# noiseinspacechannel/NIS-SAR-AMTIGMTI-Video

Hardware: AMD Instinct MI355X
Metric: focused SAR frames/sec (CSA focus, complex64) (higher is better)
Workload: dtype c64 (phase arguments f64)

## Files before the change

nis-sar-amtigmti-video_amd/csrc/api_csa.hip:

```cpp
#include "api_ctx.h"
#include "csa_kernels.h"
#include "general.h"

#include <cmath>
#include <cstdlib>
#include <string>
#include <vector>

using namespace sarx;

struct sarx_plan {
    sarx_ctx* ctx = nullptr;
    int n_az = 0, n_rg = 0;
    unsigned flags = 0;
    sarx_radar_params p{};
    int az_s = 0;
    int az_w = 32;
    int az_w_alone = 0;
    int az_impl = 1;
    int az_wpb = 4;
    int look = 0;
    float* look_slot = nullptr;
    float* look_part = nullptr;
    const float2* ati_s1 = nullptr; const float* ati_thr = nullptr; float ati_frac = 0.f; double ati_cal = 0.0;
    float *ati_phase = nullptr, *ati_m1 = nullptr, *ati_dm = nullptr; int ati_keep_image = 0;
    double2* ati_part = nullptr; int ati_nparts = 0;
    int ati_w = 32;
    float* max_slot = nullptr;
    bool az_nt = false;
    int slab_tiles = 0;
    double2 *c1 = nullptr, *c2 = nullptr, *c3 = nullptr;
    float2* buf_b = nullptr;
    float2* buf_a = nullptr;
    float2 *h_in = nullptr, *h_out = nullptr;
    static constexpr int PIPE = 2;
    float2 *pipe_in[PIPE] = {}, *pipe_out[PIPE] = {};
    int pipe_dl[PIPE] = {-1, -1};
    void* pipe_host[PIPE] = {};
    int pipe_next = 0;
    uint64_t bytes = 0;
    int mark_start = -1, mark_stop = -1;
    unsigned long long* stamp = nullptr;
    GeneralCsa* gen = nullptr;
};

static bool is_pow2(int n) { return n > 0 && (n & (n - 1)) == 0; }
static int ilog2(int n) { int l = 0; while ((1 << l) < n) ++l; return l; }

extern "C" {

static int sarx_csa_plan_create_impl(sarx_ctx* c, int n_az, int n_rg, const sarx_radar_params* prm, unsigned flags, sarx_plan** out) {
    NEED_CTX(c);
    if (!out || !prm) return fail(c, SARX_ERR_INVALID, "NULL argument");
    *out = nullptr;
    if (n_az < 2 || n_rg < 2 || n_az > 2 * TW_MAX || n_rg > 2 * TW_MAX)
        return fail(c, SARX_ERR_UNSUPPORTED, "n_az=%d n_rg=%d: sizes must be in [2, %d]", n_az, n_rg, 2 * TW_MAX);
    if (flags & ~(SARX_OUT_RG_MAJOR | SARX_FUSE_RANGE)) return fail(c, SARX_ERR_INVALID, "unknown plan flags 0x%x", flags);
    const bool general = !is_pow2(n_az) || !is_pow2(n_rg) || n_az < 16 || n_rg < 16 || n_az > TW_MAX || n_rg > TW_MAX;
    if (!(prm->sample_rate_hz > 0) || !(prm->prf_hz > 0) || !(prm->platform_speed_mps > 0) ||
        !(prm->wavelength_m > 0) || prm->chirp_rate_hz_s == 0.0)
        return fail(c, SARX_ERR_INVALID, "radar parameters must be positive (chirp rate non-zero)");
    sarx_plan* p = new sarx_plan();
    p->ctx = c; p->n_az = n_az; p->n_rg = n_rg; p->flags = flags; p->p = *prm;
    if (general) {
        std::string err;
        p->gen = general_csa_create(n_az, n_rg, prm, c->tw_all, err, true, c->cus);
        if (!p->gen) { delete p; return fail(c, SARX_ERR_UNSUPPORTED, "n_az=%d n_rg=%d: %s", n_az, n_rg, err.c_str()); }
        p->bytes = general_csa_bytes(p->gen);
        if (flags & SARX_OUT_RG_MAJOR) {
            hipError_t e2 = hipMalloc(&p->buf_a, (size_t)n_az * n_rg * sizeof(float2));
            if (e2 != hipSuccess) { int rc = fail(c, SARX_ERR_NOMEM, "hipMalloc: %s", hipGetErrorString(e2)); sarx_csa_plan_destroy(p); return rc; }
            p->bytes += (size_t)n_az * n_rg * sizeof(float2);
        }
        *out = p;
        return SARX_OK;
    }
    p->az_s = (n_az <= 128) ? n_az : (1 << (ilog2(n_az) / 2));
    p->az_w = (n_rg % 32 == 0) ? 32 : 16;
    p->az_nt = (size_t)n_az * n_rg * sizeof(float2) >= ((size_t)1 << 29);
    if (const char* e = getenv("SARX_AZ_NT")) p->az_nt = atoi(e) != 0;
    if (const char* e = getenv("SARX_SLAB_MIB")) {
        const double mib = atof(e);
        const double tile_mib = (double)p->az_s * n_rg * sizeof(float2) / (1024.0 * 1024.0);
        if (mib > 0 && p->az_s != n_az) {
            int q = (int)(mib / tile_mib);
            if (q < 1) q = 1;
            if (q > n_az / p->az_s) q = n_az / p->az_s;
            p->slab_tiles = q;
        }
    }
    if (const char* e = getenv("SARX_AZ_W")) { const int w = atoi(e); if ((w == 16 || w == 32 || w == 64) && n_rg % w == 0) p->az_w = w; }
    else if (n_rg % 64 == 0 && (size_t)n_az * n_rg * sizeof(float2) >= ((size_t)1 << 31)) p->az_w_alone = 64;
    if (const char* e = getenv("SARX_AZ_IMPL")) p->az_impl = atoi(e) != 0;
    if (const char* e = getenv("SARX_AZ_WAVES")) { const int w = atoi(e); if (w == 1 || w == 4) p->az_wpb = w; }

    const double lam = prm->wavelength_m, Kr = prm->chirp_rate_hz_s, Vr = prm->platform_speed_mps, Rref = prm->range_ref_m;
    const double fa_step = 1.0 / ((double)n_az * (1.0 / prm->prf_hz));
    std::vector<double2> c1(n_az), c2(n_az), c3(n_az);
    for (int i = 0; i < n_az; ++i) {
        const int ks = (i < n_az / 2) ? i : i - n_az;
        const double fa = (double)ks * fa_step;
        const double u = lam * fa / (2.0 * Vr);
        double arg = 1.0 - u * u;
        if (arg < 0) arg = 1e-9;
        const double D = sqrt(arg);
        const double Cs = 1.0 / D - 1.0;
        const double tau_ref = 2.0 * Rref / (C_LIGHT * D);
        c1[i] = make_double2(-0.5 * Kr * Cs, tau_ref);
        c2[i] = make_double2(0.5 / (Kr * (1.0 + Cs)), 2.0 * Rref * Cs / C_LIGHT);
        c3[i] = make_double2(C_LIGHT * D / lam, -0.5 * Kr * Cs * (1.0 + Cs));
    }
    const size_t tb = (size_t)n_az * sizeof(double2), img = (size_t)n_az * n_rg * sizeof(float2);
    auto bail = [&](hipError_t e, const char* what) {
        int rc = fail(c, e == hipErrorOutOfMemory ? SARX_ERR_NOMEM : SARX_ERR_DEVICE, "%s: %s", what, hipGetErrorString(e));
        sarx_csa_plan_destroy(p);
        return rc;
    };
    hipError_t e;
    if ((e = hipMalloc(&p->c1, tb)) != hipSuccess) return bail(e, "hipMalloc c1");
    if ((e = hipMalloc(&p->c2, tb)) != hipSuccess) return bail(e, "hipMalloc c2");
    if ((e = hipMalloc(&p->c3, tb)) != hipSuccess) return bail(e, "hipMalloc c3");
    if ((e = hipMemcpy(p->c1, c1.data(), tb, hipMemcpyHostToDevice)) != hipSuccess) return bail(e, "upload c1");
    if ((e = hipMemcpy(p->c2, c2.data(), tb, hipMemcpyHostToDevice)) != hipSuccess) return bail(e, "upload c2");
    if ((e = hipMemcpy(p->c3, c3.data(), tb, hipMemcpyHostToDevice)) != hipSuccess) return bail(e, "upload c3");
    if ((e = hipMalloc(&p->buf_b, img)) != hipSuccess) return bail(e, "hipMalloc scratch image");
    p->bytes = 3 * tb + img;
    if (flags & SARX_OUT_RG_MAJOR) {
        if ((e = hipMalloc(&p->buf_a, img)) != hipSuccess) return bail(e, "hipMalloc second scratch image");
        p->bytes += img;
    }
    *out = p;
    return SARX_OK;
}
int sarx_csa_plan_create(sarx_ctx* c, int n_az, int n_rg, const sarx_radar_params* prm, unsigned flags, sarx_plan** out) {
    return guarded(c, [&] { return sarx_csa_plan_create_impl(c, n_az, n_rg, prm, flags, out); });
}

int sarx_csa_plan_destroy(sarx_plan* p) {
    if (!p) return SARX_OK;
    hipSetDevice(p->ctx->device);
    sync_all_lanes(p->ctx);
    general_csa_destroy(p->gen);
    hipFree(p->c1); hipFree(p->c2); hipFree(p->c3);
    hipFree(p->ati_part);
    hipFree(p->buf_a); hipFree(p->buf_b); hipFree(p->h_in); hipFree(p->h_out); hipFree(p->look_part);
    for (int i = 0; i < sarx_plan::PIPE; ++i)
        if (p->pipe_dl[i] >= 0 && p->pipe_dl[i] < sarx_ctx::DL_SLOTS) { sarx_memcpy_d2h_end(p->ctx, p->pipe_dl[i]); p->pipe_dl[i] = -1; }
    if (p->ctx->dl_stream) hipStreamSynchronize(p->ctx->dl_stream);
    for (int i = 0; i < sarx_plan::PIPE; ++i) { hipFree(p->pipe_in[i]); hipFree(p->pipe_out[i]); }
    delete p;
    return SARX_OK;
}

int sarx_csa_plan_mark_range(sarx_plan* p, int slot_start, int slot_stop) {
    if (!p) return fail(nullptr, SARX_ERR_INVALID, "plan is NULL");
    if (slot_start >= N_EVENTS || slot_stop >= N_EVENTS) return fail(p->ctx, SARX_ERR_INVALID, "event slot out of range");
    p->mark_start = slot_start; p->mark_stop = slot_stop;
    return SARX_OK;
}

int sarx_csa_plan_stamp_range(sarx_plan* p, uint64_t* d_pair) {
    if (!p) return fail(nullptr, SARX_ERR_INVALID, "plan is NULL");
    if (((uintptr_t)d_pair) & 7) return fail(p->ctx, SARX_ERR_INVALID, "the stamp pair must be 8-byte aligned");
    p->stamp = reinterpret_cast<unsigned long long*>(d_pair);
    return SARX_OK;
}

int sarx_csa_plan_set_look_slot(sarx_plan* p, int looks, float* d_slot) {
    if (!p) return fail(nullptr, SARX_ERR_INVALID, "plan is NULL");
    sarx_ctx* c = p->ctx;
    hipSetDevice(c->device);
    if (!d_slot) { p->look_slot = nullptr; return SARX_OK; }
    if (p->gen) return fail(c, SARX_ERR_UNSUPPORTED, "the fused stack slot exists for power-of-two plans only (use sarx_multilook_dev)");
    if (looks < 1 || (looks & (looks - 1)) || looks > p->az_w || p->n_az % looks || p->n_rg % looks)
        return fail(c, SARX_ERR_UNSUPPORTED, "looks=%d must be a power of two <= %d dividing n_az=%d and n_rg=%d", looks, p->az_w, p->n_az, p->n_rg);
    if (p->look_part && p->look != looks) { hipStreamSynchronize(c->stream); hipFree(p->look_part); p->look_part = nullptr; }
    if (!p->look_part) {
        const size_t bytes = (size_t)p->n_az * (p->n_rg / looks) * sizeof(float);
        hipError_t e = hipMalloc(&p->look_part, bytes);
        if (e != hipSuccess) return fail(c, SARX_ERR_NOMEM, "hipMalloc look partials: %s", hipGetErrorString(e));
        p->bytes += bytes;
    }
    p->look = looks; p->look_slot = d_slot;
    return SARX_OK;
}

int sarx_csa_plan_set_max_slot(sarx_plan* p, float* d_max) {
    if (!p) return fail(nullptr, SARX_ERR_INVALID, "plan is NULL");
    if (p->gen && !general_csa_set_max_slot(p->gen, reinterpret_cast<unsigned*>(d_max)))
        return fail(p->ctx, SARX_ERR_UNSUPPORTED, "the fused maximum exists for power-of-two plans and 7199 x 13200 (sarx_ati_dpca_dev reduces it otherwise)");
    p->max_slot = d_max;
    return SARX_OK;
}

int sarx_csa_plan_set_ati(sarx_plan* p, const void* d_slc1, const float* d_max, float mask_frac, double cal_phase,
                          float* d_ati_phase_masked, float* d_slc1_mag, float* d_dpca_mag, int keep_image) {
    if (!p) return fail(nullptr, SARX_ERR_INVALID, "plan is NULL");
    sarx_ctx* c = p->ctx;
    hipSetDevice(c->device);
    if (!d_slc1) {
        p->ati_s1 = nullptr;
        if (p->gen) general_csa_set_ati(p->gen, nullptr);
        return SARX_OK;
    }
    if (!d_max || !d_ati_phase_masked || !d_slc1_mag || !d_dpca_mag) return fail(c, SARX_ERR_INVALID, "NULL pointer");
    if (p->gen) {
        const int parts = general_csa_ati_parts(p->gen);
        if (parts < 0 || (p->flags & SARX_OUT_RG_MAJOR))
            return fail(c, SARX_ERR_UNSUPPORTED, "the fused ATI products exist for power-of-two plans and 7199 x 13200 in the default image "
                                                 "layout (sarx_ati_dpca_dev otherwise)");
        if (!p->ati_part) {
            hipError_t e = hipMalloc(&p->ati_part, ((size_t)parts + 128) * sizeof(double2));
            if (e != hipSuccess) return fail(c, SARX_ERR_NOMEM, "hipMalloc ATI partial sums: %s", hipGetErrorString(e));
            p->bytes += (size_t)parts * sizeof(double2);
        }
        p->ati_nparts = parts;
        AtiFuse f{};
        f.s1 = (const float2*)d_slc1; f.phase = d_ati_phase_masked; f.m1 = d_slc1_mag; f.dm = d_dpca_mag; f.part = p->ati_part;
        f.thr = d_max; f.cc = (float)cos(cal_phase); f.cs = (float)sin(cal_phase); f.frac = mask_frac; f.keep_image = keep_image != 0;
        general_csa_set_ati(p->gen, &f);
        p->ati_s1 = f.s1; p->ati_thr = d_max;
        return SARX_OK;
    }
    if (p->n_rg % 32 || (p->flags & SARX_OUT_RG_MAJOR) || p->slab_tiles > 0)
        return fail(c, SARX_ERR_UNSUPPORTED, "the fused ATI products exist for power-of-two plans in the default image layout (sarx_ati_dpca_dev otherwise)");
    int w = (p->n_rg % 64 == 0) ? 64 : 32;
    if (const char* ev = getenv("SARX_ATI_W")) { const int e = atoi(ev); if ((e == 32 || e == 64) && p->n_rg % e == 0) w = e; }
    const int tpt = (p->az_s >= 16 ? p->az_s / 16 : 1) * w;
    if (tpt % 64) return fail(c, SARX_ERR_UNSUPPORTED, "n_az=%d n_rg=%d: the last azimuth launch's tiles have %d threads, the fused ATI "
                                                        "products need whole waves (sarx_ati_dpca_dev otherwise)", p->n_az, p->n_rg, tpt);
    p->ati_w = w;
    const int tiles = (p->az_s == p->n_az ? 1 : p->n_az / p->az_s) * (p->n_rg / w);
    const int waves = tpt / 64;
    if (!p->ati_part) {
        hipError_t e = hipMalloc(&p->ati_part, ((size_t)tiles * waves + 128) * sizeof(double2));
        if (e != hipSuccess) return fail(c, SARX_ERR_NOMEM, "hipMalloc ATI partial sums: %s", hipGetErrorString(e));
        p->bytes += (size_t)tiles * waves * sizeof(double2);
    }
    p->ati_nparts = tiles * waves;
    p->ati_s1 = (const float2*)d_slc1; p->ati_thr = d_max; p->ati_frac = mask_frac; p->ati_cal = cal_phase;
    p->ati_phase = d_ati_phase_masked; p->ati_m1 = d_slc1_mag; p->ati_dm = d_dpca_mag; p->ati_keep_image = keep_image != 0;
    return SARX_OK;
}

int sarx_csa_plan_bytes(const sarx_plan* p, uint64_t* out) {
    if (!p || !out) return fail(p ? p->ctx : nullptr, SARX_ERR_INVALID, "NULL argument");
    *out = p->bytes;
    return SARX_OK;
}

int sarx_csa_axes(const sarx_plan* p, double* range_axis, double* cross_range_axis) {
    if (!p) return fail(nullptr, SARX_ERR_INVALID, "plan is NULL");
    const double dt = 1.0 / p->p.sample_rate_hz;
    if (range_axis)
        for (int j = 0; j < p->n_rg; ++j) range_axis[j] = C_LIGHT * (p->p.t_start_fast_s + (double)j * dt) / 2.0;
    if (cross_range_axis) {
        double mean = 0.0;
        for (int i = 0; i < p->n_az; ++i) mean += (double)i / p->p.prf_hz;
        mean /= (double)p->n_az;
        for (int i = 0; i < p->n_az; ++i) cross_range_axis[i] = ((double)i / p->p.prf_hz - mean) * p->p.platform_speed_mps;
    }
    return SARX_OK;
}

static RangeArgs range_args(const sarx_plan* p, const void* in, void* out) {
    RangeArgs a{};
    a.in = (const float2*)in; a.out = (float2*)out;
    a.tw = p->ctx->tw_all + p->n_rg;
    a.c2 = p->c2; a.c3 = p->c3;
    a.dt = 1.0 / p->p.sample_rate_hz;
    a.df = 1.0 / ((double)p->n_rg * a.dt);
    a.t_start = p->p.t_start_fast_s;
    a.t0 = 2.0 * p->p.range_ref_m / C_LIGHT;
    a.inv_n = 1.0f / (float)p->n_rg;
    a.n_az = p->n_az;
    return a;
}

static AzArgs az_args(const sarx_plan* p, const void* in, void* out) {
    AzArgs a{};
    a.tw_n = p->ctx->tw_all + p->n_az;
    a.c1 = p->c1;
    a.dt = 1.0 / p->p.sample_rate_hz;
    a.t_start = p->p.t_start_fast_s;
    a.scale = 1.0f / (float)p->n_az;
    a.n_rg = p->n_rg;
    a.in = (const float2*)in; a.out = (float2*)out;
    a.nt = p->az_nt;
    return a;
}

static hipError_t run_range(const sarx_plan* p, int mode, const RangeArgs& a) {
    const sarx_ctx* c = p->ctx;
    const bool v2 = range_v2_supported(p->n_rg, mode) &&
                    (c->range_impl == 2 || (c->range_impl == 0 && p->n_rg >= 16384 && mode != RG_FUSED));
    if (mode == RG_FUSED && range_fused_wl_supported(p->n_rg) && (c->range_impl == 3 || c->range_impl == 0))
        return launch_range_fused_wl(a, (c->range_cus > 0 && c->range_cus < c->cus) ? c->range_cus : c->cus, c->stream,
                                     !(c->range_cus > 0 && c->range_cus < c->cus));
    return v2 ? launch_range_pass_v2(p->n_rg, mode, a, c->cus, c->stream) : launch_range_pass(p->n_rg, mode, a, c->stream);
}

static void ati_args(const sarx_plan* p, AzArgs& a) {
    a.ati_s1 = p->ati_s1; a.ati_thr = p->ati_thr; a.ati_frac = p->ati_frac;
    a.ati_cc = (float)cos(p->ati_cal); a.ati_cs = (float)sin(p->ati_cal);
    a.ati_phase = p->ati_phase; a.ati_m1 = p->ati_m1; a.ati_dm = p->ati_dm;
    a.ati_part = p->ati_part; a.ati_keep_image = p->ati_keep_image;
}
static int ati_finish(sarx_plan* p) {
    if (!p->ati_s1) return SARX_OK;
    sarx_ctx* c = p->ctx;
    HIPCHK(c, launch_ati_finish_sums(p->ati_part, p->ati_nparts, p->ati_thr, p->ati_part + p->ati_nparts, c->ati_out3_(), c->stream));
    return SARX_OK;
}
struct AzLast { int epi, w; };
static AzLast az_last(const sarx_plan* p, bool inv, int w_plain, AzArgs& a) {
    const bool look = inv && p->look_slot;
    if (look) { a.look_part = p->look_part; a.look = p->look; }
    const bool ati = inv && p->ati_s1;
    if (inv && !ati) a.max_out = reinterpret_cast<unsigned*>(p->max_slot);
    if (ati) ati_args(p, a);
    return {inv ? (ati ? AZ_EPI_SCALE_ATI : look ? AZ_EPI_SCALE_LOOK : AZ_EPI_SCALE) : AZ_EPI_PHI1, ati ? p->ati_w : look ? p->az_w : w_plain};
}
static int az_step(sarx_plan* p, bool inv, bool step_b, int S, const void* in, void* out, int q0, int nq) {
    sarx_ctx* c = p->ctx;
    const int n = p->n_az, RA = n / S;
    AzArgs a = az_args(p, in, out);
    a.q0 = q0;
    const bool alone = !(c->range_cus > 0 && c->range_cus < c->cus);
    const int w_plain = (alone && p->az_w_alone) ? p->az_w_alone : p->az_w;
    const auto wave = [&](int r, int epi) { return p->az_impl && n == 16384 && az_wave_supported(r, p->n_rg, epi, p->az_wpb); };
    if (!step_b) {
        a.tw_r = c->tw_all + RA;
        a.in_q_stride = 1; a.in_m_stride = S; a.out_q_stride = 1; a.out_m_stride = S;
        if (wave(RA, AZ_EPI_TWIDDLE)) HIPCHK(c, launch_az_wave(inv, AZ_EPI_TWIDDLE, p->az_wpb, a, nq, c->stream));
        else HIPCHK(c, launch_az_tile(RA, w_plain, inv, AZ_EPI_TWIDDLE, a, nq, c->stream));
    } else {
        a.tw_r = c->tw_all + S;
        a.in_q_stride = S; a.in_m_stride = 1; a.out_q_stride = 1; a.out_m_stride = RA;
        const AzLast l = az_last(p, inv, w_plain, a);
        if (wave(S, l.epi)) HIPCHK(c, launch_az_wave(inv, l.epi, p->az_wpb, a, nq, c->stream));
        else HIPCHK(c, launch_az_tile(S, l.w, inv, l.epi, a, nq, c->stream));
    }
    return SARX_OK;
}
static int look_finish(sarx_plan* p) {
    if (!p->look_slot || p->ati_s1) return SARX_OK;
    sarx_ctx* c = p->ctx;
    HIPCHK(c, launch_look_finish(p->look_part, p->look_slot, p->n_az / p->look, p->n_rg / p->look, p->look, c->stream));
    return SARX_OK;
}

static int az_pass(sarx_plan* p, bool inv, const void* in, void* tmp, void* out) {
    sarx_ctx* c = p->ctx;
    const int n = p->n_az, S = p->az_s;
    if (S == n) {
        AzArgs a = az_args(p, in, out);
        a.tw_r = c->tw_all + n;
        a.in_q_stride = 0; a.in_m_stride = 1; a.out_q_stride = 0; a.out_m_stride = 1;
        const AzLast l = az_last(p, inv, p->az_w, a);
        HIPCHK(c, launch_az_tile(n, l.w, inv, l.epi, a, 1, c->stream));
        return SARX_OK;
    }
    int rc;
    if ((rc = az_step(p, inv, false, S, in, tmp, 0, S)) != SARX_OK) return rc;
    return az_step(p, inv, true, S, tmp, out, 0, n / S);
}

int sarx_csa_pass(sarx_plan* p, int pass_id, const void* d_in, void* d_out) {
    if (!p) return fail(nullptr, SARX_ERR_INVALID, "plan is NULL");
    sarx_ctx* c = p->ctx;
    hipSetDevice(c->device);
    if (!d_in || !d_out) return fail(c, SARX_ERR_INVALID, "NULL image pointer");
    int rc;
    if (p->gen) {
        int mode = -1;
        switch (pass_id) {
            case SARX_PASS_RG_FFT_PHI2: mode = RG_FFT_PHI2; break;
            case SARX_PASS_RG_IFFT_PHI3: mode = RG_IFFT_PHI3; break;
            case SARX_PASS_RG_FUSED_23: mode = RG_FUSED; break;
            case 100: mode = RG_FFT; break;
            case 101: mode = RG_IFFT; break;
        }
        hipError_t e = hipErrorNotSupported;
        if (mode >= 0) e = general_csa_range_pass(p->gen, mode, (const float2*)d_in, (float2*)d_out, c->stream);
        else if (pass_id == SARX_PASS_AZ_FFT_PHI1 || pass_id == SARX_PASS_AZ_IFFT) {
            if (d_in == d_out) return fail(c, SARX_ERR_INVALID, "azimuth passes are out-of-place");
            if (pass_id == SARX_PASS_AZ_IFFT && (p->max_slot || p->ati_s1))
                return fail(c, SARX_ERR_UNSUPPORTED, "the per-pass azimuth IFFT of a 7199 x 13200 plan has no max-slot / ATI epilogue: switch them off or use sarx_csa_focus_dev");
            e = general_csa_az_pass(p->gen, pass_id == SARX_PASS_AZ_IFFT, (const float2*)d_in, (float2*)d_out, c->stream);
        }
        if (e == hipErrorNotSupported)
            return fail(c, SARX_ERR_UNSUPPORTED, "per-pass entry points exist for power-of-two plans, for the range passes of n_rg = 13200 "
                                                 "and for the azimuth passes of 7199 x 13200");
        HIPCHK(c, e);
        return SARX_OK;
    }
    switch (pass_id) {
        case SARX_PASS_AZ_FFT_PHI1:
        case SARX_PASS_AZ_IFFT:
            if (d_in == d_out || d_in == p->buf_b || d_out == p->buf_b)
                return fail(c, SARX_ERR_INVALID, "azimuth passes are out-of-place");
            if (p->max_slot && !p->ati_s1 && pass_id == SARX_PASS_AZ_IFFT) HIPCHK(c, hipMemsetAsync(p->max_slot, 0, MAX_SLOT_BYTES, c->stream));
            if ((rc = az_pass(p, pass_id == SARX_PASS_AZ_IFFT, d_in, p->buf_b, d_out)) != SARX_OK) return rc;
            if (pass_id == SARX_PASS_AZ_IFFT) {
                if ((rc = look_finish(p)) != SARX_OK) return rc;
                if ((rc = ati_finish(p)) != SARX_OK) return rc;
            }
            return SARX_OK;
        case SARX_PASS_RG_FFT_PHI2: { RangeArgs a = range_args(p, d_in, d_out); HIPCHK(c, run_range(p, RG_FFT_PHI2, a)); return SARX_OK; }
        case SARX_PASS_RG_IFFT_PHI3: { RangeArgs a = range_args(p, d_in, d_out); HIPCHK(c, run_range(p, RG_IFFT_PHI3, a)); return SARX_OK; }
        case SARX_PASS_RG_FUSED_23: { RangeArgs a = range_args(p, d_in, d_out); HIPCHK(c, run_range(p, RG_FUSED, a)); return SARX_OK; }
        case SARX_PASS_RG_FFT_PHI2_PERM:
        case SARX_PASS_RG_IFFT_PHI3_PERM: {
            if (!range_wp_supported(p->n_rg)) return fail(c, SARX_ERR_UNSUPPORTED, "the permuted-spectrum range passes exist for n_rg = 16384 only");
            RangeArgs a = range_args(p, d_in, d_out);
            HIPCHK(c, launch_range_wp(pass_id == SARX_PASS_RG_FFT_PHI2_PERM ? RG_FFT_PHI2 : RG_IFFT_PHI3, a, c->cus, c->stream));
            return SARX_OK;
        }
        case 110: case 111: case 112: case 113: {
            if (p->az_s == p->n_az || d_in == d_out || d_in == p->buf_b || d_out == p->buf_b)
                return fail(c, SARX_ERR_INVALID, "azimuth steps exist for four-step plans and are out-of-place");
            const bool inv = pass_id >= 112, step_b = pass_id & 1;
            if (inv && step_b && p->max_slot && !p->ati_s1) HIPCHK(c, hipMemsetAsync(p->max_slot, 0, MAX_SLOT_BYTES, c->stream));
            return az_step(p, inv, step_b, p->az_s, d_in, d_out, 0, step_b ? p->n_az / p->az_s : p->az_s);
        }
        case 100: { RangeArgs a = range_args(p, d_in, d_out); HIPCHK(c, run_range(p, RG_FFT, a)); return SARX_OK; }
        case 101: { RangeArgs a = range_args(p, d_in, d_out); HIPCHK(c, run_range(p, RG_IFFT, a)); return SARX_OK; }
    }
    return fail(c, SARX_ERR_INVALID, "unknown pass id %d", pass_id);
}

int sarx_csa_focus_dev(sarx_plan* p, const void* d_phist, void* d_image) {
    if (!p) return fail(nullptr, SARX_ERR_INVALID, "plan is NULL");
    sarx_ctx* c = p->ctx;
    hipSetDevice(c->device);
    if (!d_phist || !d_image || d_phist == d_image) return fail(c, SARX_ERR_INVALID, "image pointers NULL or aliased");
    if (p->ati_s1 && (d_image == (const void*)p->ati_s1 || d_phist == (const void*)p->ati_s1))
        return fail(c, SARX_ERR_INVALID, "the first channel's image (sarx_csa_plan_set_ati) must not be this focus's input or output: the output buffer is scratch");
    const bool rg_major = p->flags & SARX_OUT_RG_MAJOR;
    int rc;
    if (p->max_slot && !p->ati_s1) HIPCHK(c, hipMemsetAsync(p->max_slot, 0, MAX_SLOT_BYTES, c->stream));
    if (p->gen) {
        float2* dst = rg_major ? p->buf_a : (float2*)d_image;
        HIPCHK(c, general_csa_focus(p->gen, (const float2*)d_phist, dst, c->stream));
        if ((rc = ati_finish(p)) != SARX_OK) return rc;
        if (rg_major) HIPCHK(c, launch_corner_turn(p->buf_a, (float2*)d_image, p->n_az, p->n_rg, c->stream));
        return SARX_OK;
    }
    if (p->slab_tiles > 0 && p->az_s != p->n_az && (p->flags & SARX_FUSE_RANGE)) {
        const int S = p->az_s, RA = p->n_az / S, Q = p->slab_tiles;
        float2* last = rg_major ? p->buf_a : (float2*)d_image;
        if ((rc = az_step(p, false, false, S, d_phist, d_image, 0, S)) != SARX_OK) return rc;
        bool marked = false;
        for (int q0 = 0; q0 < RA; q0 += Q) {
            const int nq = (q0 + Q <= RA) ? Q : RA - q0;
            if ((rc = az_step(p, false, true, S, d_image, p->buf_b, q0, nq)) != SARX_OK) return rc;
            RangeArgs a = range_args(p, p->buf_b, p->buf_b);
            a.n_az = nq * S; a.row0 = q0; a.row_inner = nq; a.row_stride = RA;
            const bool mark = !marked && p->mark_start >= 0;
            if (mark) { HIPCHK(c, hipEventRecord(c->ev[p->mark_start], c->stream)); c->ev_set[p->mark_start] = true; }
            HIPCHK(c, run_range(p, RG_FUSED, a));
            if (mark && p->mark_stop >= 0) { HIPCHK(c, hipEventRecord(c->ev[p->mark_stop], c->stream)); c->ev_set[p->mark_stop] = true; marked = true; }
            if ((rc = az_step(p, true, false, RA, p->buf_b, p->buf_b, q0, nq)) != SARX_OK) return rc;
        }
        if ((rc = az_step(p, true, true, RA, p->buf_b, last, 0, S)) != SARX_OK) return rc;
        if ((rc = look_finish(p)) != SARX_OK) return rc;
        if (rg_major) HIPCHK(c, launch_corner_turn(p->buf_a, (float2*)d_image, p->n_az, p->n_rg, c->stream));
        return SARX_OK;
    }
    if ((rc = az_pass(p, false, d_phist, d_image, p->buf_b)) != SARX_OK) return rc;
    if (p->mark_start >= 0) { HIPCHK(c, hipEventRecord(c->ev[p->mark_start], c->stream)); c->ev_set[p->mark_start] = true; }
    if (p->flags & SARX_FUSE_RANGE) {
        RangeArgs a = range_args(p, p->buf_b, p->buf_b);
        a.stamp = p->stamp;
        HIPCHK(c, run_range(p, RG_FUSED, a));
    } else if (range_wp_supported(p->n_rg) && (c->range_impl == 0 || c->range_impl == 4)) {
        RangeArgs a = range_args(p, p->buf_b, p->buf_b);
        HIPCHK(c, launch_range_wp(RG_FFT_PHI2, a, c->cus, c->stream));
        HIPCHK(c, launch_range_wp(RG_IFFT_PHI3, a, c->cus, c->stream));
    } else {
        RangeArgs a = range_args(p, p->buf_b, p->buf_b);
        HIPCHK(c, run_range(p, RG_FFT_PHI2, a));
        HIPCHK(c, run_range(p, RG_IFFT_PHI3, a));
    }
    if (p->mark_stop >= 0) { HIPCHK(c, hipEventRecord(c->ev[p->mark_stop], c->stream)); c->ev_set[p->mark_stop] = true; }
    float2* last = rg_major ? p->buf_a : (float2*)d_image;
    if (p->az_s == p->n_az) {
        if ((rc = az_pass(p, true, p->buf_b, nullptr, last)) != SARX_OK) return rc;
    } else {
        if ((rc = az_pass(p, true, p->buf_b, p->buf_b, last)) != SARX_OK) return rc;
    }
    if ((rc = look_finish(p)) != SARX_OK) return rc;
    if ((rc = ati_finish(p)) != SARX_OK) return rc;
    if (rg_major) HIPCHK(c, launch_corner_turn(p->buf_a, (float2*)d_image, p->n_az, p->n_rg, c->stream));
    return SARX_OK;
}


int sarx_csa_focus_host_c128(sarx_plan* p, const void* phist_host, void* image_host) {
    if (!p) return fail(nullptr, SARX_ERR_INVALID, "plan is NULL");
    sarx_ctx* c = p->ctx;
    hipSetDevice(c->device);
    if (!phist_host || !image_host) return fail(c, SARX_ERR_INVALID, "NULL host pointer");
    const size_t img = (size_t)p->n_az * p->n_rg * sizeof(float2);
    if (!p->h_in) { hipError_t e = hipMalloc(&p->h_in, img); if (e != hipSuccess) return fail(c, SARX_ERR_NOMEM, "hipMalloc staging: %s", hipGetErrorString(e)); }
    if (!p->h_out) { hipError_t e = hipMalloc(&p->h_out, img); if (e != hipSuccess) return fail(c, SARX_ERR_NOMEM, "hipMalloc staging: %s", hipGetErrorString(e)); }
    HIPCHK(c, staged_copy(c, p->h_in, phist_host, img, true, true));
    int rc = sarx_csa_focus_dev(p, p->h_in, p->h_out);
    if (rc != SARX_OK) return rc;
    HIPCHK(c, staged_copy(c, image_host, p->h_out, img, false));
    return SARX_OK;
}

int sarx_csa_focus_host(sarx_plan* p, const void* phist_host, void* image_host) {
    if (!p) return fail(nullptr, SARX_ERR_INVALID, "plan is NULL");
    sarx_ctx* c = p->ctx;
    hipSetDevice(c->device);
    if (!phist_host || !image_host) return fail(c, SARX_ERR_INVALID, "NULL host pointer");
    const size_t img = (size_t)p->n_az * p->n_rg * sizeof(float2);
    if (!p->h_in) { hipError_t e = hipMalloc(&p->h_in, img); if (e != hipSuccess) return fail(c, SARX_ERR_NOMEM, "hipMalloc staging: %s", hipGetErrorString(e)); }
    if (!p->h_out) { hipError_t e = hipMalloc(&p->h_out, img); if (e != hipSuccess) return fail(c, SARX_ERR_NOMEM, "hipMalloc staging: %s", hipGetErrorString(e)); }
    HIPCHK(c, staged_copy(c, p->h_in, phist_host, img, true));
    int rc = sarx_csa_focus_dev(p, p->h_in, p->h_out);
    if (rc != SARX_OK) return rc;
    HIPCHK(c, staged_copy(c, image_host, p->h_out, img, false));
    return SARX_OK;
}

int sarx_csa_focus_host_begin(sarx_plan* p, const void* phist_host, void* image_host, int* out_ticket) {
    if (!p) return fail(nullptr, SARX_ERR_INVALID, "plan is NULL");
    sarx_ctx* c = p->ctx;
    hipSetDevice(c->device);
    if (!phist_host || !image_host || !out_ticket) return fail(c, SARX_ERR_INVALID, "NULL pointer");
    *out_ticket = -1;
    const int s = p->pipe_next;
    if (p->pipe_dl[s] != -1) return fail(c, SARX_ERR_INVALID, "%d frames are in flight on this plan: call sarx_csa_focus_host_end first", sarx_plan::PIPE);
    const size_t img = (size_t)p->n_az * p->n_rg * sizeof(float2);
    for (float2** b : {&p->pipe_in[s], &p->pipe_out[s]})
        if (!*b) { hipError_t e = hipMalloc(b, img); if (e != hipSuccess) return fail(c, SARX_ERR_NOMEM, "hipMalloc pipeline buffer: %s", hipGetErrorString(e)); }
    HIPCHK(c, staged_copy(c, p->pipe_in[s], phist_host, img, true, false, false));
    int rc = sarx_csa_focus_dev(p, p->pipe_in[s], p->pipe_out[s]);
    if (rc != SARX_OK) return rc;
    if (is_page_locked(image_host)) {
        int slot = -1;
        if ((rc = sarx_memcpy_d2h_begin(c, image_host, p->pipe_out[s], img, &slot)) != SARX_OK) {
            hipStreamSynchronize(c->stream);
            return rc;
        }
        p->pipe_dl[s] = slot; p->pipe_host[s] = nullptr;
    } else {
        p->pipe_dl[s] = sarx_ctx::DL_SLOTS; p->pipe_host[s] = image_host;
    }
    p->pipe_next = (s + 1) % sarx_plan::PIPE;
    *out_ticket = s;
    return SARX_OK;
}
int sarx_csa_focus_host_end(sarx_plan* p, int ticket) {
    if (!p) return fail(nullptr, SARX_ERR_INVALID, "plan is NULL");
    sarx_ctx* c = p->ctx;
    hipSetDevice(c->device);
    if (ticket < 0 || ticket >= sarx_plan::PIPE || p->pipe_dl[ticket] == -1) return fail(c, SARX_ERR_INVALID, "ticket %d is not in flight", ticket);
    const int slot = p->pipe_dl[ticket];
    p->pipe_dl[ticket] = -1;
    if (slot == sarx_ctx::DL_SLOTS) {
        const size_t img = (size_t)p->n_az * p->n_rg * sizeof(float2);
        HIPCHK(c, staged_copy(c, p->pipe_host[ticket], p->pipe_out[ticket], img, false));
        return SARX_OK;
    }
    return sarx_memcpy_d2h_end(c, slot);
}

}
```

nis-sar-amtigmti-video_amd/csrc/csa_kernels.h:

```cpp
#pragma once
#include <hip/hip_runtime.h>
#include <stddef.h>
#include <stdint.h>

namespace sarx {

enum RangeMode { RG_FFT = 0, RG_IFFT = 1, RG_FFT_PHI2 = 2, RG_IFFT_PHI3 = 3, RG_FUSED = 4,
                 RG_CONV = 5 };
enum AzEpilogue { AZ_EPI_NONE = 0, AZ_EPI_TWIDDLE = 1, AZ_EPI_PHI1 = 2, AZ_EPI_SCALE = 3,
                  AZ_EPI_TWCOL = 4,
                  AZ_EPI_PROCOL = 5,
                  AZ_EPI_ROWVEC = 6,
                  AZ_EPI_TWIDDLE_PADIN = 7,
                  AZ_EPI_CROPOUT = 8,
                  AZ_EPI_TWIDDLE_ROWSIN = 9,
                  AZ_EPI_SCALE_ROWSOUT = 10,
                  AZ_EPI_CROPOUT_PHI1 = 11,
                  AZ_EPI_CROPOUT_MAG = 12,
                  AZ_EPI_SCALE_LOOK = 13,
                  AZ_EPI_SCALE_ATI = 14 };

struct RangeArgs {
    const float2* in;
    float2* out;
    const float2* tw;
    const double2* c2;
    const double2* c3;
    double df;
    double dt;
    double t_start;
    double t0;
    float inv_n;
    int n_az;
    const float2* mulvec;
    int mul_period;
    int row0, row_inner, row_stride;
    int conv_valid, conv_crop0, conv_out;
    size_t conv_in_ld, conv_out_ld;
    int conv_wrap_n, conv_wrap_c0;
    unsigned long long* stamp;
};
__host__ __device__ inline int range_row(const RangeArgs& a, int line) {
    return a.row_inner ? a.row0 + line % a.row_inner + (line / a.row_inner) * a.row_stride : line;
}

constexpr unsigned MAX_SHARDS = 256;
constexpr size_t MAX_SLOT_BYTES = MAX_SHARDS * 32 * sizeof(float);
struct AzArgs {
    const float2* in;
    float2* out;
    const float2* tw_r;
    const float2* tw_n;
    const double2* c1;
    const float2* rowvec;
    size_t io_ld;
    int io_rows, io_cols;
    int io_shift_in;
    float hamming_inv;
    int io_shift_out;
    float* out_mag;
    bool nt;
    float* look_part;
    int look;
    const float2* ati_s1; float *ati_phase, *ati_m1, *ati_dm; double2* ati_part; const float* ati_thr;
    float ati_cc, ati_cs, ati_frac; int ati_keep_image;
    unsigned* max_out;
    int valid_len;
    double dt, t_start;
    float scale;
    float tw_scale;
    int n_rg;
    int in_q_stride, in_m_stride, out_q_stride, out_m_stride;
    int q0;
};

inline int persistent_grid(int wgs_per_cu, int cus, int work_items) {
    if (wgs_per_cu < 1) wgs_per_cu = 1;
    if (cus < 1) cus = 1;
    long long g = (long long)wgs_per_cu * cus;
    if (g > work_items) g = work_items;
    if (g < 1) g = 1;
    return (int)g;
}

hipError_t launch_range_pass(int n_rg, int mode, const RangeArgs& a, hipStream_t st);
bool range_v2_supported(int n_rg, int mode);
hipError_t launch_range_pass_v2(int n_rg, int mode, const RangeArgs& a, int cus, hipStream_t st);
bool range_fused_wl_supported(int n_rg);
hipError_t launch_range_fused_wl(const RangeArgs& a, int cus, hipStream_t st, bool alone = false);
bool range_mixed_supported(int n_rg);
hipError_t launch_range_mixed(int n_rg, int mode, const RangeArgs& a, int cus, hipStream_t st);
bool range_conv_supported(int m);
hipError_t launch_range_conv(int m, const RangeArgs& a, int cus, hipStream_t st);
hipError_t launch_az_tile(int r, int w, bool inv, int epi, const AzArgs& a, int nq, hipStream_t st);
bool az_wave_supported(int r, int n_rg, int epi, int wpb);
hipError_t launch_az_wave(bool inv, int epi, int wpb, const AzArgs& a, int nq, hipStream_t st);

hipError_t launch_az_conv(int s, int ra, const AzArgs& a, hipStream_t st);

struct AtiFuse {
    const float2* s1;
    float *phase, *m1, *dm;
    double2* part;
    const float* thr;
    float cc, cs, frac;
    int keep_image;
};
struct PfaArgs {
    const float2* in; size_t in_ld; int in_cols;
    float2* u; size_t u_ld; int u_cols;
    float2* out; size_t out_ld; int out_cols;
    const unsigned* offin; const unsigned* offu;
    unsigned off0in, off0u;
    unsigned pitch_u, pitch_out;
    const float2* bspec;
    const double2* c1; double dt, t_start;
    float scale;
    int c1k, c2k;
    bool nt;
    unsigned* max_out;
    AtiFuse ati;
};
struct AzPfa;
bool az_pfa_supported(int n_az);
AzPfa* az_pfa_create(size_t in_ld, size_t u_ld, size_t out_ld, hipError_t* err);
void az_pfa_destroy(AzPfa* z);
hipError_t az_pfa_run(const AzPfa* z, bool inv, const float2* src, size_t src_ld, int src_cols, float2* u, size_t u_ld,
                      float2* dst, size_t dst_ld, int dst_cols, int epi, const double2* c1, double dt, double t_start,
                      float scale, hipStream_t st, unsigned* max_out = nullptr, const AtiFuse* ati = nullptr);
int az_pfa_ati_parts(int dst_cols);

bool az_pfa7200_supported(int n);
hipError_t az_pfa7200_run(bool inv, const float2* src, size_t src_ld, int cols, float2* u, size_t u_ld, float2* dst, float* dst_mag,
                          size_t dst_ld, int shift_in, int shift_out, const float* pre, float scale, hipStream_t st);
bool range_wp_supported(int n_rg);
hipError_t launch_range_wp(int mode, const RangeArgs& a, int cus, hipStream_t st);

struct AtiArgs {
    const float2* s1;
    const float2* s2;
    size_t n;
    float cal_c, cal_s;
    float* ati_phase;
    float* mag1;
    float* dpca_mag;
    float2* interf;
    float2* diff;
    float* mag2;
    float* ph1;
    float* ph2;
    float* dpca_phase;
    bool nt;
    const float* thr_max;
    float mask_frac;
    float* part_max;
    double2* part_sum;
};
int ati_blocks(size_t n);
hipError_t launch_ati_dpca(const AtiArgs& a, hipStream_t st);
hipError_t launch_ati_finish(const float* part_max, const double2* part_sum, int blocks, double* out3, hipStream_t st);
hipError_t launch_ati_finish_sums(const double2* part_sum, int n, const float* max_shards, double2* scratch, double* out3, hipStream_t st);
hipError_t launch_mask_phase(const float* phase, const float* mag, size_t n, float thr, float* out, hipStream_t st);
hipError_t launch_mask_phase_frac(const float* phase, const float* mag, size_t n, float frac, const double* out3, float* out,
                                  hipStream_t st);
hipError_t launch_magnitude(const float2* in, float* out, size_t n, hipStream_t st);
hipError_t launch_spin(int blocks, unsigned long long cycles, unsigned* sink, hipStream_t st);
hipError_t launch_max_abs_f32(const float* x, size_t n, float* out, hipStream_t st);
hipError_t launch_corner_turn(const float2* in, float2* out, int rows, int cols, hipStream_t st);
hipError_t launch_multilook(const float2* in, float* out, int rows, int cols, int looks, hipStream_t st);
hipError_t launch_look_finish(const float* part, float* out, int out_rows, int cols, int looks, hipStream_t st);
hipError_t launch_fill_noise(float2* buf, size_t n, uint64_t seed, hipStream_t st);

hipError_t launch_ocean_noise(float2* buf, size_t n, float sigma, float clutter_power, float nu, uint64_t seed, hipStream_t st,
                              const float* levels = nullptr);
hipError_t launch_noise_levels(const double* part, int blocks, size_t n, int ref_is_max, double snr_lin, double scr_lin, float* levels,
                               hipStream_t st);
hipError_t launch_power_stats(const float2* buf, size_t n, double* part, int blocks, hipStream_t st);

struct EchoArgs {
    const double2* tau_pb;
    const float* amp;
    const float* amp_pt;
    const double* t_fast;
    float2* out;
    double kr, t_p, u_off;
    int n_pulses, n_targets, n_samples;
    int accumulate;
};
hipError_t launch_echo_synth(const EchoArgs& a, hipStream_t st);
struct EchoGeoArgs {
    int model;
    int n_pulses, n_targets;
    const double* tgt_pos;
    const double* tgt_vel;
    const double* t_pulse;
    const double* tx_pos;
    const double* aux;
    const double* rcs;
    double c, fc, l_ant, lambda;
    double2* tau_pb;
    float* amp_pt;
};
hipError_t launch_echo_geometry(const EchoGeoArgs& a, hipStream_t st);

}
```

nis-sar-amtigmti-video_amd/csrc/range_fused_wl.hip:

```cpp
#include <cstdlib>
#include "csa_kernels.h"
#include "fft_core.hpp"
#include "phase.hpp"

namespace sarx {

namespace wl {
constexpr int N = 16384, M = 1024, THREADS = 512;
constexpr int ROWSTR = LdsSize<M, 1>::value;
constexpr size_t LDS_BYTES = (size_t)16 * ROWSTR * sizeof(cf);

__device__ __forceinline__ int pad32(int idx) { return idx + (idx >> 5); }

__device__ __forceinline__ void cross_fwd32(cf* v, int t, int w, int l, cf* lds, bool lead_barrier) {
    if (lead_barrier) __syncthreads();
#pragma unroll
    for (int q = 0; q < 16; ++q)
        *reinterpret_cast<float4*>(&lds[q * ROWSTR + 2 * t]) = make_float4(v[q].x, v[q].y, v[16 + q].x, v[16 + q].y);
    __syncthreads();
    const cf* line = lds + (2 * w + (l >> 5)) * ROWSTR + (l & 31);
#pragma unroll
    for (int r = 0; r < 32; ++r) v[r] = line[32 * r];
}
__device__ __forceinline__ void cross_inv32(cf* v, int t, int w, int l, cf* lds) {
    cf* line = lds + (2 * w + (l >> 5)) * ROWSTR + (l & 31);
#pragma unroll
    for (int r = 0; r < 32; ++r) line[32 * r] = v[r];
    __syncthreads();
#pragma unroll
    for (int q = 0; q < 16; ++q) {
        const float4 p = *reinterpret_cast<const float4*>(&lds[q * ROWSTR + 2 * t]);
        v[q] = make_float2(p.x, p.y);
        v[16 + q] = make_float2(p.z, p.w);
    }
}
template <bool INV> __device__ __forceinline__ void sub1024_r32(cf* v, int i, cf* img, const cf* wp) {
    dft32<INV>(v);
    exchange_sync<true>();
#pragma unroll
    for (int r = 0; r < 32; ++r) img[pad32(32 * i + r)] = v[r];
    exchange_sync<true>();
#pragma unroll
    for (int r = 0; r < 32; ++r) v[r] = img[pad32(i + 32 * r)];
#pragma unroll
    for (int r = 1; r < 32; ++r)
        v[r] = INV ? make_float2(fmaf(v[r].x, wp[r].x, v[r].y * wp[r].y), fmaf(v[r].y, wp[r].x, -v[r].x * wp[r].y))
                   : cmul(v[r], wp[r]);
    dft32<INV>(v);
}
}

template <int PF>
__device__ __forceinline__ void range_fused_wl_body(const RangeArgs& a) {
    using namespace wl;
    constexpr bool TOUCH = (PF == 1);
    extern __shared__ __attribute__((aligned(16))) char smem_raw[];
    cf* lds = reinterpret_cast<cf*>(smem_raw);
    if (a.stamp && threadIdx.x == 0) atomicMin(a.stamp, (unsigned long long)__builtin_amdgcn_s_memrealtime());
    const cf* __restrict__ tw = a.tw;
    const cf* __restrict__ tw_m = a.tw - N + M;

    cf wp[32];
    {
        const cf w1 = stage_twiddle<M, M, false>((int)(threadIdx.x & 31), tw_m);
        wp[0] = make_float2(1.f, 0.f);
        wp[1] = w1;
#pragma unroll
        for (int r = 2; r < 32; ++r) wp[r] = cmul(wp[r / 2], wp[r - r / 2]);
    }
    cf cw[2][16];
#pragma unroll
    for (int b = 0; b < 2; ++b) {
        const cf w1 = stage_twiddle<N, N, false>(2 * (int)threadIdx.x + b, tw);
        cw[b][0] = make_float2(1.f, 0.f);
        cw[b][1] = w1;
#pragma unroll
        for (int q = 2; q < 16; ++q) cw[b][q] = cmul(cw[b][q / 2], cw[b][q - q / 2]);
    }
    unsigned pf0 = 0, pf1 = 0;
    for (int line = blockIdx.x; line < a.n_az; line += gridDim.x) {
        const int row = range_row(a, line);
        int t = threadIdx.x;
        asm volatile("" : "+v"(t));
        const int w = t >> 6, l = t & 63;
        cf* __restrict__ dst = a.out + (size_t)row * N;

        cf v[32];
        const cf* __restrict__ src = a.in + (size_t)row * N;
#pragma unroll
        for (int r = 0; r < 16; ++r) {
            const float4 q4 = ld16<false>(src + 2 * t + r * M);
            v[r] = make_float2(q4.x, q4.y);
            v[16 + r] = make_float2(q4.z, q4.w);
        }
        auto touch_next = [&] {
            const int nl = line + (int)gridDim.x;
            if (nl < a.n_az) {
                const cf* np = a.in + (size_t)range_row(a, nl) * N + 16 * t;
                asm volatile("global_load_dword %0, %2, off\n\tglobal_load_dword %1, %3, off"
                             : "=&v"(pf0), "=&v"(pf1) : "v"(np), "v"(np + 16 * THREADS) : "memory");
            }
        };
        const double2 c2 = sload_double2(a.c2 + row), c3 = sload_double2(a.c3 + row);
#pragma unroll
        for (int b = 0; b < 2; ++b) {
            dft16<false>(v + 16 * b);
#pragma unroll
            for (int q = 1; q < 16; ++q) v[16 * b + q] = cmul(v[16 * b + q], cw[b][q]);
        }
        cf* img = lds + (2 * w + (l >> 5)) * ROWSTR;
        const int li = l & 31;
        if constexpr (TOUCH) {
            asm volatile("" :: "v"(pf0), "v"(pf1), "v"(v[0].x), "v"(v[31].y));
        }
        cross_fwd32(v, t, w, l, lds, line != (int)blockIdx.x);
        if constexpr (TOUCH) touch_next();
        sub1024_r32<false>(v, li, img, wp);
        {
#pragma unroll
            for (int half = 0; half < 2; ++half) {
                FixPhase q0 = phi2_seed(2 * w + (l >> 5) + 16 * li + half * (8192 - N), 512, c2, a.df);
#pragma unroll
                for (int rr = 0; rr < 16; ++rr) v[half * 16 + rr] = cmul(v[half * 16 + rr], q0.next());
            }
        }
        sub1024_r32<true>(v, li, img, wp);
        exchange_sync<true>();
        cross_inv32(v, t, w, l, lds);
#pragma unroll
        for (int b = 0; b < 2; ++b) {
#pragma unroll
            for (int q = 1; q < 16; ++q) {
                const cf x = v[16 * b + q], c = cw[b][q];
                v[16 * b + q] = make_float2(fmaf(x.x, c.x, x.y * c.y), fmaf(x.y, c.x, -x.x * c.y));
            }
            dft16<true>(v + 16 * b);
        }
        {
            const float sc = a.inv_n;
            FixPhase q0 = phi3_seed(2 * t, M, c3, a.dt, a.t_start, a.t0);
            FixPhase q1 = phi3_seed(2 * t + 1, M, c3, a.dt, a.t_start, a.t0);
#pragma unroll
            for (int n1 = 0; n1 < 16; ++n1) {
                cf p0 = q0.next(), p1 = q1.next();
                p0.x *= sc; p0.y *= sc; p1.x *= sc; p1.y *= sc;
                const cf y0 = cmul(v[n1], p0), y1 = cmul(v[16 + n1], p1);
                st16<false>(dst + 2 * t + n1 * M, make_float4(y0.x, y0.y, y1.x, y1.y));
            }
        }
    }
    if constexpr (TOUCH) {
        __builtin_amdgcn_s_waitcnt(0x0F70);
        asm volatile("" :: "v"(pf0), "v"(pf1));
    }
    if (a.stamp && threadIdx.x == 0) {
        __builtin_amdgcn_s_waitcnt(0x0F70);
        atomicMax(a.stamp + 1, (unsigned long long)__builtin_amdgcn_s_memrealtime());
    }
}
__global__ __launch_bounds__(wl::THREADS, 2) void range_fused_wl_kernel(RangeArgs a) { range_fused_wl_body<0>(a); }
__global__ __launch_bounds__(wl::THREADS, 2) void range_fused_wl_touch_kernel(RangeArgs a) { range_fused_wl_body<1>(a); }

bool range_fused_wl_supported(int n_rg) { return n_rg == wl::N; }

hipError_t launch_range_fused_wl(const RangeArgs& a, int cus, hipStream_t st, bool alone) {
    static const int pf = [] { const char* e = getenv("SARX_WL_PREFETCH"); return e ? atoi(e) : -1; }();
    const bool touch = pf < 0 ? (alone && a.in == a.out) : pf == 1;
    auto k = touch ? range_fused_wl_touch_kernel : range_fused_wl_kernel;
    hipError_t e = hipFuncSetAttribute(reinterpret_cast<const void*>(k), hipFuncAttributeMaxDynamicSharedMemorySize, (int)wl::LDS_BYTES);
    if (e != hipSuccess) return e;
    const int grid = persistent_grid(1, cus, a.n_az);
    hipLaunchKernelGGL(k, dim3(grid), dim3(wl::THREADS), wl::LDS_BYTES, st, a);
    return hipGetLastError();
}

}
```

Before: 253.6.

## Stage next range line into LDS with async global-to-LDS loads

Adds a staged form of the fused 16384-point range kernel. Each block issues global_load_lds_dwordx4 copies of its next azimuth line into LDS while it finishes the current line, then reads the input from LDS instead of global memory. The goal is to hide global load latency behind the FFT and chirp compute. The default launch now uses the staged form, with non-temporal loads when the kernel runs alone. New pass ids let each form be tested separately. This relies on careful vmcnt/lgkmcnt waits and on LDS reuse between the exchange buffers and the staged row, which risks hazards and extra waits.

```diff
diff --git a/nis-sar-amtigmti-video_amd/csrc/api_csa.hip b/nis-sar-amtigmti-video_amd/csrc/api_csa.hip
--- a/nis-sar-amtigmti-video_amd/csrc/api_csa.hip
+++ b/nis-sar-amtigmti-video_amd/csrc/api_csa.hip
@@ -290,13 +290,13 @@
     return a;
 }
 
-static hipError_t run_range(const sarx_plan* p, int mode, const RangeArgs& a) {
+static hipError_t run_range(const sarx_plan* p, int mode, const RangeArgs& a, int wl_form = WL_AUTO) {
     const sarx_ctx* c = p->ctx;
     const bool v2 = range_v2_supported(p->n_rg, mode) &&
                     (c->range_impl == 2 || (c->range_impl == 0 && p->n_rg >= 16384 && mode != RG_FUSED));
     if (mode == RG_FUSED && range_fused_wl_supported(p->n_rg) && (c->range_impl == 3 || c->range_impl == 0))
         return launch_range_fused_wl(a, (c->range_cus > 0 && c->range_cus < c->cus) ? c->range_cus : c->cus, c->stream,
-                                     !(c->range_cus > 0 && c->range_cus < c->cus));
+                                     !(c->range_cus > 0 && c->range_cus < c->cus), wl_form);
     return v2 ? launch_range_pass_v2(p->n_rg, mode, a, c->cus, c->stream) : launch_range_pass(p->n_rg, mode, a, c->stream);
 }
 
@@ -427,6 +427,16 @@
         case 100: { RangeArgs a = range_args(p, d_in, d_out); HIPCHK(c, run_range(p, RG_FFT, a)); return SARX_OK; }
         case 101: { RangeArgs a = range_args(p, d_in, d_out); HIPCHK(c, run_range(p, RG_IFFT, a)); return SARX_OK; }
     }
+    if (pass_id > 0 && (pass_id & 0xff) >= 120 && (pass_id & 0xff) <= 122) {
+        const int lines = pass_id >> 8;
+        if (!range_fused_wl_supported(p->n_rg) || !(c->range_impl == 3 || c->range_impl == 0))
+            return fail(c, SARX_ERR_UNSUPPORTED, "the forms of the fused range launch exist for n_rg = 16384 only");
+        if (lines > p->n_az) return fail(c, SARX_ERR_INVALID, "pass id %d: %d lines of a plan of %d", pass_id, lines, p->n_az);
+        RangeArgs a = range_args(p, d_in, d_out);
+        if (lines) a.n_az = lines;
+        HIPCHK(c, run_range(p, RG_FUSED, a, (pass_id & 0xff) - 120 + WL_PLAIN));
+        return SARX_OK;
+    }
     return fail(c, SARX_ERR_INVALID, "unknown pass id %d", pass_id);
 }
 
diff --git a/nis-sar-amtigmti-video_amd/csrc/csa_kernels.h b/nis-sar-amtigmti-video_amd/csrc/csa_kernels.h
--- a/nis-sar-amtigmti-video_amd/csrc/csa_kernels.h
+++ b/nis-sar-amtigmti-video_amd/csrc/csa_kernels.h
@@ -87,7 +87,8 @@
 bool range_v2_supported(int n_rg, int mode);
 hipError_t launch_range_pass_v2(int n_rg, int mode, const RangeArgs& a, int cus, hipStream_t st);
 bool range_fused_wl_supported(int n_rg);
-hipError_t launch_range_fused_wl(const RangeArgs& a, int cus, hipStream_t st, bool alone = false);
+enum { WL_AUTO = -1, WL_PLAIN = 0, WL_TOUCH = 1, WL_STAGED = 2 };
+hipError_t launch_range_fused_wl(const RangeArgs& a, int cus, hipStream_t st, bool alone = false, int form = WL_AUTO);
 bool range_mixed_supported(int n_rg);
 hipError_t launch_range_mixed(int n_rg, int mode, const RangeArgs& a, int cus, hipStream_t st);
 bool range_conv_supported(int m);
diff --git a/nis-sar-amtigmti-video_amd/csrc/range_fused_wl.hip b/nis-sar-amtigmti-video_amd/csrc/range_fused_wl.hip
--- a/nis-sar-amtigmti-video_amd/csrc/range_fused_wl.hip
+++ b/nis-sar-amtigmti-video_amd/csrc/range_fused_wl.hip
@@ -48,15 +48,49 @@
                    : cmul(v[r], wp[r]);
     dft32<INV>(v);
 }
+
+template <int R, bool NT>
+__device__ __forceinline__ void stage_piece(const cf* row_s, unsigned voff, unsigned lds_w) {
+    unsigned keep;
+    const cf* g = row_s + R * M;
+    const unsigned d = lds_w + (unsigned)(R * ROWSTR * sizeof(cf));
+    if constexpr (NT)
+        asm volatile("s_mov_b32 %0, m0\n\ts_mov_b32 m0, %3\n\ts_nop 4\n\tglobal_load_lds_dwordx4 %1, %2 nt\n\ts_mov_b32 m0, %0"
+                     : "=&s"(keep) : "v"(voff), "s"(g), "s"(d) : "memory");
+    else
+        asm volatile("s_mov_b32 %0, m0\n\ts_mov_b32 m0, %3\n\ts_nop 4\n\tglobal_load_lds_dwordx4 %1, %2\n\ts_mov_b32 m0, %0"
+                     : "=&s"(keep) : "v"(voff), "s"(g), "s"(d) : "memory");
+}
+struct StageAddr { const cf* row_s; unsigned voff, lds_w; };
+__device__ __forceinline__ StageAddr stage_addr(const cf* in, int row, int t, const cf* lds) {
+    const unsigned long long pv = (unsigned long long)(in + (size_t)row * N);
+    StageAddr s;
+    s.row_s = reinterpret_cast<const cf*>(((unsigned long long)(unsigned)__builtin_amdgcn_readfirstlane((int)(pv >> 32)) << 32) |
+                                          (unsigned)__builtin_amdgcn_readfirstlane((int)(unsigned)pv));
+    s.voff = (unsigned)t * 16u;
+    const unsigned lds0 = (unsigned)(unsigned long long)(__attribute__((address_space(3))) const char*)lds;
+    s.lds_w = lds0 + (unsigned)__builtin_amdgcn_readfirstlane(t >> 6) * (unsigned)(128 * sizeof(cf));
+    return s;
+}
+template <int R0, int R1, bool NT> __device__ __forceinline__ void stage_pieces(const StageAddr& s) {
+    if constexpr (R0 < R1) {
+        stage_piece<R0, NT>(s.row_s, s.voff, s.lds_w);
+        stage_pieces<R0 + 1, R1, NT>(s);
+    }
+}
 }
 
 template <int PF>
 __device__ __forceinline__ void range_fused_wl_body(const RangeArgs& a) {
     using namespace wl;
-    constexpr bool TOUCH = (PF == 1);
+    constexpr bool TOUCH = (PF & 1) != 0, STAGED = (PF & 2) != 0, NT = TOUCH && STAGED;
     extern __shared__ __attribute__((aligned(16))) char smem_raw[];
     cf* lds = reinterpret_cast<cf*>(smem_raw);
     if (a.stamp && threadIdx.x == 0) atomicMin(a.stamp, (unsigned long long)__builtin_amdgcn_s_memrealtime());
+    if constexpr (STAGED) {
+        if ((int)blockIdx.x < a.n_az)
+            stage_pieces<0, 16, NT>(stage_addr(a.in, range_row(a, (int)blockIdx.x), (int)threadIdx.x, lds));
+    }
     const cf* __restrict__ tw = a.tw;
     const cf* __restrict__ tw_m = a.tw - N + M;
 
@@ -78,6 +112,7 @@
         for (int q = 2; q < 16; ++q) cw[b][q] = cmul(cw[b][q / 2], cw[b][q - q / 2]);
     }
     unsigned pf0 = 0, pf1 = 0;
+    if constexpr (STAGED) asm volatile("s_waitcnt vmcnt(0)" ::: "memory");
     for (int line = blockIdx.x; line < a.n_az; line += gridDim.x) {
         const int row = range_row(a, line);
         int t = threadIdx.x;
@@ -87,11 +122,21 @@
 
         cf v[32];
         const cf* __restrict__ src = a.in + (size_t)row * N;
-#pragma unroll
-        for (int r = 0; r < 16; ++r) {
-            const float4 q4 = ld16<false>(src + 2 * t + r * M);
-            v[r] = make_float2(q4.x, q4.y);
-            v[16 + r] = make_float2(q4.z, q4.w);
+        if constexpr (STAGED) {
+            asm volatile("s_waitcnt vmcnt(16)" ::: "memory");
+#pragma unroll
+            for (int r = 0; r < 16; ++r) {
+                const float4 q4 = *reinterpret_cast<const float4*>(&lds[r * ROWSTR + 2 * t]);
+                v[r] = make_float2(q4.x, q4.y);
+                v[16 + r] = make_float2(q4.z, q4.w);
+            }
+        } else {
+#pragma unroll
+            for (int r = 0; r < 16; ++r) {
+                const float4 q4 = ld16<false>(src + 2 * t + r * M);
+                v[r] = make_float2(q4.x, q4.y);
+                v[16 + r] = make_float2(q4.z, q4.w);
+            }
         }
         auto touch_next = [&] {
             const int nl = line + (int)gridDim.x;
@@ -127,6 +172,11 @@
         sub1024_r32<true>(v, li, img, wp);
         exchange_sync<true>();
         cross_inv32(v, t, w, l, lds);
+        if constexpr (STAGED) {
+            asm volatile("s_waitcnt lgkmcnt(0)" ::: "memory");
+            const int nl = line + (int)gridDim.x;
+            if (nl < a.n_az) stage_pieces<0, 16, NT>(stage_addr(a.in, range_row(a, nl), t, lds));
+        }
 #pragma unroll
         for (int b = 0; b < 2; ++b) {
 #pragma unroll
@@ -158,15 +208,16 @@
         atomicMax(a.stamp + 1, (unsigned long long)__builtin_amdgcn_s_memrealtime());
     }
 }
-__global__ __launch_bounds__(wl::THREADS, 2) void range_fused_wl_kernel(RangeArgs a) { range_fused_wl_body<0>(a); }
-__global__ __launch_bounds__(wl::THREADS, 2) void range_fused_wl_touch_kernel(RangeArgs a) { range_fused_wl_body<1>(a); }
+__global__ __launch_bounds__(wl::THREADS, 2) void range_fused_wl_kernel(RangeArgs a) { range_fused_wl_body<2>(a); }
+__global__ __launch_bounds__(wl::THREADS, 2) void range_fused_wl_plain_kernel(RangeArgs a) { range_fused_wl_body<0>(a); }
+__global__ __launch_bounds__(wl::THREADS, 2) void range_fused_wl_touch_kernel(RangeArgs a) { range_fused_wl_body<3>(a); }
 
 bool range_fused_wl_supported(int n_rg) { return n_rg == wl::N; }
 
-hipError_t launch_range_fused_wl(const RangeArgs& a, int cus, hipStream_t st, bool alone) {
+hipError_t launch_range_fused_wl(const RangeArgs& a, int cus, hipStream_t st, bool alone, int form) {
     static const int pf = [] { const char* e = getenv("SARX_WL_PREFETCH"); return e ? atoi(e) : -1; }();
-    const bool touch = pf < 0 ? (alone && a.in == a.out) : pf == 1;
-    auto k = touch ? range_fused_wl_touch_kernel : range_fused_wl_kernel;
+    if (form == WL_AUTO) form = (pf >= WL_PLAIN && pf <= WL_STAGED) ? pf : alone ? WL_TOUCH : WL_STAGED;
+    auto k = form == WL_PLAIN ? range_fused_wl_plain_kernel : form == WL_TOUCH ? range_fused_wl_touch_kernel : range_fused_wl_kernel;
     hipError_t e = hipFuncSetAttribute(reinterpret_cast<const void*>(k), hipFuncAttributeMaxDynamicSharedMemorySize, (int)wl::LDS_BYTES);
     if (e != hipSuccess) return e;
     const int grid = persistent_grid(1, cus, a.n_az);
```

Result: no change. 254.7, median of 6 (+0.4%).
